# ikt-luh/Unified-Point-Cloud-Compression

Hardware: AMD Instinct MI355X
Metric: points/sec encode+decode, longdress vox10, 1 GPU; bpp & D1-PSNR parity (higher is better)
Workload: dtype f32

## Files before the change

unified_point_cloud_compression_amd/csrc/pcc_conv.hip:

```cpp
#include <vector>

#include "pcc_common.h"

typedef float f32x16 __attribute__((ext_vector_type(16)));

static constexpr int LDS_LD = 36;
static constexpr int MAXK = 128;
static constexpr int MAXK_T = 512;

enum { MODE_CONV = 0, MODE_GDN = 1, MODE_IGDN = 2 };
#ifdef PCC_DBG_BUILD
#define PCC_DBG_ON(a, bit) (((a).dbg & (bit)) != 0)
#else
#define PCC_DBG_ON(a, bit) false
#endif
__device__ inline float act1(float v, int act, float slope);

struct ConvArgs {
  const float* feat;
  const float* wp;
  const float* bias;
  const int* hdr;
  const int* nbr;
  const int* rows;
  float* out;
  long long n_out;
  long long n_in;
  long long wp_elems;
  const int* pair_in = nullptr;
  const int* tile_k = nullptr;
  const long long* n_tiles = nullptr;
  const unsigned char* featb = nullptr;
  int ksplit = 1;
  float* part = nullptr;
  int dbg = 0;
  int nt = 0;
  bool wh_ok = false;
  const unsigned char* feath = nullptr;
  const float* frow_inv = nullptr;
  int arith = PCC_ARITH_H3;
  int* guard = nullptr;
  float guard_lim = 0.f;
  int cin, cout, cout_pad;
  int cb_log2;
  int ppo;
  int act;
  float slope;
};

__host__ __device__ inline int bn_for(int cout) { return cout >= 128 ? 128 : (cout > 32 ? 64 : 32); }

static constexpr unsigned BUF_OOB = 0xFFFF0000u;
static constexpr long long BUF_MAX_BYTES = 0xFFFE0000ll;

template <int WM, int WN, int TM, int TN, int MODE, bool BUF>
__global__ void __launch_bounds__(256) k_conv_mfma(ConvArgs a) {
  constexpr int BM = WM * TM * 32;
  constexpr int BN = WN * TN * 32;
  static_assert(WM * WN == 4, "4 waves per workgroup");
  __shared__ __attribute__((aligned(16))) float As[BM * LDS_LD];
  __shared__ __attribute__((aligned(16))) float Bs[BN * LDS_LD];
  __shared__ unsigned char act_flag[MAXK];
  __shared__ unsigned char act_list[MAXK];
  __shared__ unsigned char act_kid[MAXK];
  __shared__ int s_nact;

  const int tid = threadIdx.x, lane = tid & 63, w = tid >> 6;

  const int cpx = gridDim.x >> 3;
  const int wid = (blockIdx.x & 7) * cpx + (blockIdx.x >> 3);
  const int gy = a.cout_pad / BN;
  int tile_id = wid / gy;
  int colblock = (wid - tile_id * gy) * BN;
  if (a.hdr == nullptr && a.pair_in == nullptr && gy > 8) {
    const int g = wid / (8 * gy), rem = wid - g * 8 * gy;
    colblock = (rem >> 3) * BN;
    tile_id = g * 8 + (rem & 7);
  }

  int pos0, npos, k_count, koff_begin;
  long long seg_pos_count;
  const int* seg_nbr = nullptr;
  const bool pair_mode = (a.pair_in != nullptr);
  bool identity = (a.hdr == nullptr) && !pair_mode;
  if (pair_mode) {
// ... 3278 lines not shown
    prof_note(PCC_FORM_GATHER_CSR, 0.0, 0.0);
    prof_push();
  }
  return PCC_OK;
}

extern "C" int pcc_convt_fwd_csr(const float* feat_in, int64_t n_in, int32_t cin, const float* packed_w,
                                 const float* bias, int32_t K, int32_t cout, const int32_t* first,
                                 const int32_t* pair_ids, int64_t n_out, float* T, float* out, int32_t act, float slope,
                                 const int32_t* ex_nbr, int32_t ex_K, const float* ex_bias, int32_t arith, int32_t* d_guard,
                                 void* stream) {
  return convt_fwd_csr_impl(feat_in, n_in, cin, packed_w, bias, K, cout, first, pair_ids, n_out, T, out, act, slope, ex_nbr,
                            ex_K, ex_bias, nullptr, nullptr, arith, d_guard, stream);
}

static int ilog2_i(int v) { int l = 0; while ((1 << l) < v) ++l; return l; }
static PccGrid grid_from_host(const uint64_t* bits, const int32_t* rank, const int32_t* h) {
  PccGrid g;
  g.bits = (const unsigned long long*)bits; g.rank = rank;
  for (int i = 0; i < 3; ++i) { g.lo[i] = h[i]; g.dims[i] = h[3 + i]; }
  g.ts_log2 = ilog2_i(h[6]); g.nbatch = h[7];
  return g;
}

extern "C" int pcc_convt_fwd_csr_grid(const float* feat_in, int64_t n_in, int32_t cin, const float* packed_w,
                                      const float* bias, int32_t K, int32_t cout, const int32_t* first,
                                      const int32_t* pair_ids, int64_t n_out, float* T, float* out, int32_t act, float slope,
                                      const int64_t* out_keys, const uint64_t* out_bits, const int32_t* out_rank,
                                      const int32_t* h_out, const float* ex_bias, const int32_t* wg_end, int32_t arith,
                                      int32_t* d_guard, void* stream) {
  PCC_REQUIRE(out_keys && out_bits && out_rank && h_out && ex_bias, "pcc_convt_fwd_csr_grid: NULL array");
  const PccGrid ex = grid_from_host(out_bits, out_rank, h_out);
  return convt_fwd_csr_impl(feat_in, n_in, cin, packed_w, bias, K, cout, first, pair_ids, n_out, T, out, act, slope,
                            nullptr, 27, ex_bias, &ex, (const long long*)out_keys, arith, d_guard, stream, wg_end);
}

struct ThinGridArgs {
  const float* t; const float* bias; const long long* keys; PccGrid g; float* out; long long n; int cout;
};

template <int COUT_MAX>
__global__ void __launch_bounds__(256) k_thin_gather_grid(ThinGridArgs a) {
  const long long p = (long long)blockIdx.x * 256 + threadIdx.x;
  if (p >= a.n) return;
  const PccGrid& g = a.g;
  const long long key = a.keys[p];
  const int b = (int)(key >> 48);
  const int cx = (((int)((key >> 32) & 0xFFFF) - (int)PCC_BIAS - g.lo[0]) >> g.ts_log2);
  const int cy = (((int)((key >> 16) & 0xFFFF) - (int)PCC_BIAS - g.lo[1]) >> g.ts_log2);
  const int cz = (((int)(key & 0xFFFF) - (int)PCC_BIAS - g.lo[2]) >> g.ts_log2);
  const int z_lo = cz > 0 ? cz - 1 : 0, z_hi = cz + 1 < g.dims[2] ? cz + 1 : g.dims[2] - 1;
  const int nz = z_hi - z_lo + 1;
  float acc[COUT_MAX];
#pragma unroll
  for (int o = 0; o < COUT_MAX; ++o) acc[o] = 0.f;
#pragma unroll
  for (int c = 0; c < 9; ++c) {
    const int nx = cx + c % 3 - 1, ny = cy + c / 3 - 1;
    if (nx < 0 || ny < 0 || nx >= g.dims[0] || ny >= g.dims[1]) continue;
    const long long cell = (((long long)b * g.dims[0] + nx) * g.dims[1] + ny) * g.dims[2] + z_lo;
    const long long wi = cell >> 6;
    const int sh = (int)(cell & 63);
    const unsigned long long w0 = g.bits[wi];
    unsigned long long f64 = w0 >> sh;
    if (sh + nz > 64) f64 |= g.bits[wi + 1] << (64 - sh);
    unsigned f = (unsigned)f64 & ((1u << nz) - 1u);
    if (!f) continue;
    int r = g.rank[wi] + __popcll(w0 & ((1ull << sh) - 1ull));
    while (f) {
      const int t = __ffs((int)f) - 1;
      f &= f - 1;
      const int k = c + 9 * (z_lo + t - cz + 1);
#pragma unroll
      for (int o = 0; o < COUT_MAX; ++o)
        if (o < a.cout) acc[o] += a.t[(long long)(k * a.cout + o) * a.n + r];
      ++r;
    }
  }
#pragma unroll
  for (int o = 0; o < COUT_MAX; ++o)
    if (o < a.cout) a.out[p * a.cout + o] = acc[o] + (a.bias ? a.bias[o] : 0.f);
}

__global__ void __launch_bounds__(256) k_thin_gather_grid1(ThinGridArgs a) {
  const long long p = (long long)blockIdx.x * 256 + threadIdx.x;
  if (p >= a.n) return;
  const PccGrid& g = a.g;
  const long long key = a.keys[p];
  const int b = (int)(key >> 48);
  const int cx = (((int)((key >> 32) & 0xFFFF) - (int)PCC_BIAS - g.lo[0]) >> g.ts_log2);
  const int cy = (((int)((key >> 16) & 0xFFFF) - (int)PCC_BIAS - g.lo[1]) >> g.ts_log2);
  const int cz = (((int)(key & 0xFFFF) - (int)PCC_BIAS - g.lo[2]) >> g.ts_log2);
  const int z_lo = cz > 0 ? cz - 1 : 0, z_hi = cz + 1 < g.dims[2] ? cz + 1 : g.dims[2] - 1;
  const int nz = z_hi - z_lo + 1;
  const int dz0 = z_lo - cz + 1;
  unsigned long long w0[9], w1[9];
  int rk[9], sh[9];
  bool ok[9];
#pragma unroll
  for (int c = 0; c < 9; ++c) {
    const int nx = cx + c % 3 - 1, ny = cy + c / 3 - 1;
    ok[c] = !(nx < 0 || ny < 0 || nx >= g.dims[0] || ny >= g.dims[1]);
    const long long cell = ok[c] ? (((long long)b * g.dims[0] + nx) * g.dims[1] + ny) * g.dims[2] + z_lo : 0ll;
    const long long wi = cell >> 6;
    sh[c] = (int)(cell & 63);
    w0[c] = g.bits[wi];
    rk[c] = g.rank[wi];
    w1[c] = (sh[c] + nz > 64) ? g.bits[wi + 1] : 0ull;
  }
  const __amdgpu_buffer_rsrc_t rsT = __builtin_amdgcn_make_buffer_rsrc(const_cast<float*>(a.t), (short)0,
                                                                       (int)(unsigned)((size_t)27 * a.n * 4), 0x00020000);
  float v[27];
#pragma unroll
  for (int c = 0; c < 9; ++c) {
    unsigned long long f64 = w0[c] >> sh[c];
    if (sh[c] + nz > 64) f64 |= w1[c] << (64 - sh[c]);
    const unsigned f = ok[c] ? ((unsigned)f64 & ((1u << nz) - 1u)) : 0u;
    const int r = rk[c] + __popcll(w0[c] & ((1ull << sh[c]) - 1ull));
#pragma unroll
    for (int t = 0; t < 3; ++t) {
      const int k = c + 9 * (dz0 + t);
      const unsigned row = (unsigned)(r + __popc(f & ((1u << t) - 1u)));
      const unsigned off = ((f >> t) & 1u) ? ((unsigned)k * (unsigned)a.n + row) * 4u : BUF_OOB;
      v[c * 3 + t] = __builtin_bit_cast(float, __builtin_amdgcn_raw_buffer_load_b32(rsT, off, 0, 0));
    }
  }
  float acc = 0.f;
#pragma unroll
  for (int i = 0; i < 27; ++i) acc += v[i];
  a.out[p] = acc + (a.bias ? a.bias[0] : 0.f);
}

template <int CIN>
__global__ void __launch_bounds__(256) k_thin_project_z(const float* __restrict__ feat, const long long* __restrict__ keys,
                                                        long long n_in, long long ts, const float* __restrict__ wt,
                                                        float* __restrict__ t) {
  extern __shared__ __attribute__((aligned(16))) float w_s[];
  __shared__ float sd[27][258];
  for (int i = threadIdx.x; i < 27 * CIN; i += 256) w_s[i] = wt[i];
  __syncthreads();
  const long long base = (long long)blockIdx.x * 256;
  const long long i = base + threadIdx.x;
  const bool valid = i < n_in;
  float4 x[CIN / 4];
#pragma unroll
  for (int c = 0; c < CIN / 4; ++c) x[c] = valid ? reinterpret_cast<const float4*>(feat + i * CIN)[c] : make_float4(0.f, 0.f, 0.f, 0.f);
  const long long key = valid ? keys[i] : -(1ll << 62);
  const bool adjm = valid && i > 0 && keys[i - 1] == key - ts;
  const bool adjp = valid && i + 1 < n_in && keys[i + 1] == key + ts;
#pragma unroll 1
  for (int k = 0; k < 27; ++k) {
    float acc = 0.f;
#pragma unroll
    for (int c = 0; c < CIN / 4; ++c) {
      const float4 w = reinterpret_cast<const float4*>(w_s + k * CIN)[c];
      acc += x[c].x * w.x + x[c].y * w.y + x[c].z * w.z + x[c].w * w.w;
    }
    sd[k][1 + threadIdx.x] = acc;
  }
  if (threadIdx.x < 18) {
    const int e = threadIdx.x < 9 ? threadIdx.x : threadIdx.x - 9;
    const long long r = threadIdx.x < 9 ? base - 1 : base + 256;
    const int k = threadIdx.x < 9 ? e : e + 18;
    float acc = 0.f;
    if (r >= 0 && r < n_in) {
#pragma unroll
      for (int c = 0; c < CIN / 4; ++c) {
        const float4 xv = reinterpret_cast<const float4*>(feat + r * CIN)[c];
        const float4 w = reinterpret_cast<const float4*>(w_s + k * CIN)[c];
        acc += xv.x * w.x + xv.y * w.y + xv.z * w.z + xv.w * w.w;
      }
    }
    sd[k][threadIdx.x < 9 ? 0 : 257] = acc;
  }
  __syncthreads();
  if (!valid) return;
  const int col = 1 + threadIdx.x;
#pragma unroll 1
  for (int g = 0; g < 9; ++g) {
    const float lo = sd[g][col], mid = sd[g + 9][col], hi = sd[g + 18][col];
    const float from_dn = sd[g][col - 1];
    const float from_up = sd[g + 18][col + 1];
    t[(long long)g * n_in + i] = (mid + (adjm ? from_dn : 0.f)) + (adjp ? from_up : 0.f);
    t[(long long)(9 + g) * n_in + i] = lo;
    t[(long long)(18 + g) * n_in + i] = hi;
  }
}

__global__ void __launch_bounds__(256) k_thin_gather_grid1z(ThinGridArgs a) {
  const long long p = (long long)blockIdx.x * 256 + threadIdx.x;
  if (p >= a.n) return;
  const PccGrid& g = a.g;
  const long long key = a.keys[p];
  const int b = (int)(key >> 48);
  const int cx = (((int)((key >> 32) & 0xFFFF) - (int)PCC_BIAS - g.lo[0]) >> g.ts_log2);
  const int cy = (((int)((key >> 16) & 0xFFFF) - (int)PCC_BIAS - g.lo[1]) >> g.ts_log2);
  const int cz = (((int)(key & 0xFFFF) - (int)PCC_BIAS - g.lo[2]) >> g.ts_log2);
  const int z_lo = cz > 0 ? cz - 1 : 0, z_hi = cz + 1 < g.dims[2] ? cz + 1 : g.dims[2] - 1;
  const int nz = z_hi - z_lo + 1;
  const int dz0 = z_lo - cz + 1;
  unsigned long long w0[9], w1[9];
  int rk[9], sh[9];
  bool ok[9];
#pragma unroll
  for (int c = 0; c < 9; ++c) {
    const int nx = cx + c % 3 - 1, ny = cy + c / 3 - 1;
    ok[c] = !(nx < 0 || ny < 0 || nx >= g.dims[0] || ny >= g.dims[1]);
    const long long cell = ok[c] ? (((long long)b * g.dims[0] + nx) * g.dims[1] + ny) * g.dims[2] + z_lo : 0ll;
    const long long wi = cell >> 6;
    sh[c] = (int)(cell & 63);
    w0[c] = g.bits[wi];
    rk[c] = g.rank[wi];
    w1[c] = (sh[c] + nz > 64) ? g.bits[wi + 1] : 0ull;
  }
  const __amdgpu_buffer_rsrc_t rsT = __builtin_amdgcn_make_buffer_rsrc(const_cast<float*>(a.t), (short)0,
                                                                       (int)(unsigned)((size_t)27 * a.n * 4), 0x00020000);
  const int tm = 1 - dz0;
  float v[27];
#pragma unroll
  for (int c = 0; c < 9; ++c) {
    unsigned long long f64 = w0[c] >> sh[c];
    if (sh[c] + nz > 64) f64 |= w1[c] << (64 - sh[c]);
    const unsigned f = ok[c] ? ((unsigned)f64 & ((1u << nz) - 1u)) : 0u;
    const unsigned r = (unsigned)(rk[c] + __popcll(w0[c] & ((1ull << sh[c]) - 1ull)));
    const bool mid = (f >> tm) & 1u;
    const bool low = dz0 == 0 && (f & 1u);
    const int tu = 2 - dz0;
    const bool upp = tu < nz && ((f >> tu) & 1u);
    const unsigned row_mid = r + __popc(f & ((1u << tm) - 1u));
    const unsigned row_up = r + __popc(f & ((1u << tu) - 1u));
    const unsigned n = (unsigned)a.n;
    const unsigned o_s = mid ? ((unsigned)c * n + row_mid) * 4u : BUF_OOB;
    const unsigned o_u = (!mid && low) ? ((unsigned)(9 + c) * n + r) * 4u : BUF_OOB;
    const unsigned o_d = (!mid && upp) ? ((unsigned)(18 + c) * n + row_up) * 4u : BUF_OOB;
    v[c * 3 + 0] = __builtin_bit_cast(float, __builtin_amdgcn_raw_buffer_load_b32(rsT, o_s, 0, 0));
    v[c * 3 + 1] = __builtin_bit_cast(float, __builtin_amdgcn_raw_buffer_load_b32(rsT, o_u, 0, 0));
    v[c * 3 + 2] = __builtin_bit_cast(float, __builtin_amdgcn_raw_buffer_load_b32(rsT, o_d, 0, 0));
  }
  float acc = 0.f;
#pragma unroll
  for (int i = 0; i < 27; ++i) acc += v[i];
  a.out[p] = acc + (a.bias ? a.bias[0] : 0.f);
}

static long long g_thin_z_min_rows = 1ll << 20;
extern "C" int pcc_set_thin_z_min_rows(int64_t rows) { g_thin_z_min_rows = rows; return PCC_OK; }

extern "C" size_t pcc_thin_grid_ws_bytes(int64_t n, int32_t cout) { return (size_t)27 * cout * (size_t)(n > 0 ? n : 1) * sizeof(float) + 256; }

extern "C" int pcc_conv_thin_grid_fwd(const float* feat, int64_t n, int32_t cin, const float* packed_w ,
                                      const float* bias, int32_t cout, const int64_t* keys, const uint64_t* bits,
                                      const int32_t* rank, const int32_t* h_grid, float* out, void* ws, size_t ws_bytes,
                                      void* stream) {
  hipStream_t s = (hipStream_t)stream;
  if (n <= 0) return PCC_OK;
  PCC_REQUIRE(feat && packed_w && keys && bits && rank && h_grid && out && ws, "pcc_conv_thin_grid_fwd: NULL array");
  PCC_REQUIRE(cout >= 1 && cout <= 4 && conv_kind(27, cin, cout) == KIND_THIN_T, "pcc_conv_thin_grid_fwd: unsupported shape cin=%d cout=%d", cin, cout);
  if (ws_bytes < pcc_thin_grid_ws_bytes(n, cout)) { pcc_set_error("pcc_conv_thin_grid_fwd: workspace too small"); return PCC_EWS; }
  float* t = (float*)ws;
  const int kc = 27 * cout;
  if (g_thin_z_min_rows >= 0 && cout == 1 && cin == 16 && (size_t)27 * n * 4 <= (size_t)BUF_MAX_BYTES && n >= g_thin_z_min_rows) {
    k_thin_project_z<16><<<(unsigned)pcc_cdiv(n, 256), 256, (size_t)27 * 16 * sizeof(float), s>>>(
        feat, (const long long*)keys, n, (long long)h_grid[6], packed_w, t);
    ThinGridArgs az;
    az.t = t; az.bias = bias; az.keys = (const long long*)keys; az.g = grid_from_host(bits, rank, h_grid); az.out = out; az.n = n; az.cout = 1;
    k_thin_gather_grid1z<<<(unsigned)pcc_cdiv(n, 256), 256, 0, s>>>(az);
    PCC_LAUNCH_CHECK();
    return PCC_OK;
  }
  switch (cin) {
    case 4: PCC_TRY(launch_project<4>(feat, n, packed_w, kc, t, s)); break;
    case 8: PCC_TRY(launch_project<8>(feat, n, packed_w, kc, t, s)); break;
    case 16: PCC_TRY(launch_project<16>(feat, n, packed_w, kc, t, s)); break;
    case 32: PCC_TRY(launch_project<32>(feat, n, packed_w, kc, t, s)); break;
    default: PCC_TRY(launch_project<64>(feat, n, packed_w, kc, t, s)); break;
  }
  ThinGridArgs a;
  a.t = t; a.bias = bias; a.keys = (const long long*)keys; a.g = grid_from_host(bits, rank, h_grid); a.out = out; a.n = n; a.cout = cout;
  if (cout == 1 && (size_t)27 * n * 4 <= (size_t)BUF_MAX_BYTES) k_thin_gather_grid1<<<(unsigned)pcc_cdiv(n, 256), 256, 0, s>>>(a);
  else if (cout == 1) k_thin_gather_grid<1><<<(unsigned)pcc_cdiv(n, 256), 256, 0, s>>>(a);
  else k_thin_gather_grid<4><<<(unsigned)pcc_cdiv(n, 256), 256, 0, s>>>(a);
  PCC_LAUNCH_CHECK();
  return PCC_OK;
}

__global__ void k_gdn_pack(const float* __restrict__ beta_raw, const float* __restrict__ gamma_raw, int c,
                           float beta_bound, float gamma_bound, float pedestal, int cout_pad, int cb_log2,
                           float* __restrict__ packed, float* __restrict__ beta_eff) {
  const long long t = (long long)blockIdx.x * blockDim.x + threadIdx.x;
  if (t < c) {
    const float b = fmaxf(beta_raw[t], beta_bound);
    beta_eff[t] = b * b - pedestal;
  }
  const long long total = (long long)c * cout_pad;
  if (t >= total) return;
  const int CB = 1 << cb_log2;
  const int within = (int)(t & (CB - 1));
  const long long q = t >> cb_log2;
  const int col = (int)(q % cout_pad);
  const int cbi = (int)(q / cout_pad);
  const int ci = (cbi << cb_log2) + within;
  float v = 0.f;
  if (col < c) {
    const float g = fmaxf(gamma_raw[(long long)col * c + ci], gamma_bound);
    v = g * g - pedestal;
  }
  packed[t] = v;
// ... 54 lines not shown
```

unified_point_cloud_compression_amd/csrc/pcc_map.hip:

```cpp
#include <string.h>

#include "pcc_common.h"

struct SegPlan {
  int nseg;
  int K;
  int listed;
  int k_count[PCC_MAP_MAX_SEG];
  int koff_begin[PCC_MAP_MAX_SEG];
  unsigned char koffs[192];
  unsigned char order[192];
};

__device__ __forceinline__ void write_hdr(const SegPlan& plan, const int* __restrict__ class_begin, int class_stride,
                                          int64_t n_out, int* __restrict__ hdr) {
  {
    const int i = (int)threadIdx.x;
    if (i < plan.K && i < 192) {
      hdr[HDR_KOFFS + i] = plan.listed ? plan.koffs[i] : i;
      hdr[HDR_ORDER + i] = plan.order[i];
    }
  }
  if (threadIdx.x != 0) return;
  hdr[HDR_NSEG] = plan.nseg;
  hdr[HDR_K] = plan.K;
  hdr[HDR_FLAGS] = plan.listed;
  int64_t nbr_begin = 0;
  for (int s = 0; s < plan.nseg; ++s) {
    int pb = 0, pc = (int)n_out;
    if (class_begin) {
      pb = class_begin[s * class_stride];
      const int pe = (s + 1 < plan.nseg) ? class_begin[(s + 1) * class_stride] : (int)n_out;
      pc = pe - pb;
    }
    int* seg = hdr + HDR_SEG0 + s * SEG_WORDS;
    seg[SEG_POS_BEGIN] = pb;
    seg[SEG_POS_COUNT] = pc;
    seg[SEG_K_COUNT] = plan.k_count[s];
    seg[SEG_KOFF_BEGIN] = plan.koff_begin[s];
    seg[SEG_NBR_LO] = (int)(nbr_begin & 0xFFFFFFFFll);
    seg[SEG_NBR_HI] = (int)(nbr_begin >> 32);
    nbr_begin += (int64_t)pc * plan.k_count[s];
  }
}

__global__ void k_write_hdr(SegPlan plan, const int* __restrict__ class_begin, int class_stride,
                            int64_t n_out, int* __restrict__ hdr) {
  if (blockIdx.x != 0) return;
  write_hdr(plan, class_begin, class_stride, n_out, hdr);
}

static constexpr bool ORDER_Z_INNERMOST = false;
static void plan_order(SegPlan& plan, int ks) {
  for (int s = 0; s < plan.nseg; ++s) {
    const int kb = plan.koff_begin[s], kc = plan.k_count[s];
    int key[192];
    for (int j = 0; j < kc; ++j) {
      const int kid = plan.listed ? plan.koffs[kb + j] : (kb + j);
      key[j] = (kid % (ks * ks)) * ks + kid / (ks * ks);
      plan.order[kb + j] = (unsigned char)j;
    }
    if (!ORDER_Z_INNERMOST) continue;
    for (int a = 1; a < kc; ++a)
      for (int b = a; b > 0 && key[plan.order[kb + b]] < key[plan.order[kb + b - 1]]; --b) {
        const unsigned char t = plan.order[kb + b]; plan.order[kb + b] = plan.order[kb + b - 1]; plan.order[kb + b - 1] = t;
      }
  }
}

__device__ inline void count_pairs(bool hit, int* __restrict__ block_counts) {
  if (!block_counts) return;
  __shared__ int wc[4];
  const unsigned long long m = __ballot(hit);
  if ((threadIdx.x & 63) == 0) wc[threadIdx.x >> 6] = __popcll(m);
  __syncthreads();
  if (threadIdx.x == 0)
    block_counts[(int64_t)blockIdx.y * gridDim.x + blockIdx.x] = wc[0] + wc[1] + wc[2] + wc[3];
}

__global__ void __launch_bounds__(1024) k_sum_counts(const int* __restrict__ c, int64_t n,
                                                     int64_t* __restrict__ total) {
  __shared__ long long ws[16];
  long long s = 0;
  for (int64_t i = threadIdx.x; i < n; i += 1024) s += c[i];
#pragma unroll
// ... 529 lines not shown
  return PCC_OK;
}

extern "C" int pcc_coords_stride_grid(const int64_t* keys, int64_t n, const int64_t* d_n, const int32_t* h_grid, uint64_t* bits,
                                      int32_t* rank, int64_t* out_keys, int64_t* d_count, void* ws, size_t ws_bytes,
                                      void* stream) {
  hipStream_t s = (hipStream_t)stream;
  PCC_REQUIRE(h_grid && bits && rank && out_keys && d_count, "pcc_coords_stride_grid: NULL array");
  const int64_t words = pcc_grid_words(h_grid);
  PCC_REQUIRE(words >= 1 && words < (1ll << 31), "pcc_coords_stride_grid: lattice too large (%lld words)", (long long)words);
  const int P = h_grid[6];
  PCC_REQUIRE(P >= 1 && (P & (P - 1)) == 0, "pcc_coords_stride_grid: pitch must be a power of two");
  PCC_REQUIRE(h_grid[0] % P == 0 && h_grid[1] % P == 0 && h_grid[2] % P == 0,
              "pcc_coords_stride_grid: lattice origin must be a multiple of the pitch %d", P);
  if (ws_bytes < pcc_grid_ws_bytes(words)) {
    pcc_set_error("pcc_coords_stride_grid: workspace too small");
    return PCC_EWS;
  }
  PCC_CHECK_HIP(hipMemsetAsync(bits, 0, (size_t)words * 8, s));
  if (n > 0) {
    PCC_REQUIRE(keys, "pcc_coords_stride_grid: keys is NULL");
    k_grid_bits_any<<<(unsigned)pcc_cdiv(n, 256), 256, 0, s>>>(keys, n, d_n, h_grid[0], h_grid[1], h_grid[2], h_grid[3],
                                                              h_grid[4], h_grid[5], ilog2(P), (unsigned long long*)bits);
    PCC_LAUNCH_CHECK();
  }
  return grid_rank((const unsigned long long*)bits, words, rank, h_grid, ilog2(P), out_keys, d_count, ws, ws_bytes, s);
}

__global__ void k_grid_bits_each(const int64_t* __restrict__ keys, int64_t n, int lo0, int lo1, int lo2, int d0, int d1,
                                 int d2, int tsl, unsigned long long* __restrict__ bits, int64_t* __restrict__ off_lattice) {
  const int64_t i = (int64_t)blockIdx.x * blockDim.x + threadIdx.x;
  if (i >= n) return;
  const int64_t key = keys[i];
  const int x = (int)((key >> 32) & 0xFFFF) - (int)PCC_BIAS - lo0, y = (int)((key >> 16) & 0xFFFF) - (int)PCC_BIAS - lo1,
            z = (int)(key & 0xFFFF) - (int)PCC_BIAS - lo2;
  if ((x | y | z) & ((1 << tsl) - 1)) { *off_lattice = 1; return; }
  const long long c = grid_cell(key, lo0, lo1, lo2, d0, d1, d2, tsl);
  atomicOr(&bits[c >> 6], 1ull << (c & 63));
}

__global__ void k_grid_first_user(const int64_t* __restrict__ keys, int64_t n, int lo0, int lo1, int lo2, int d0, int d1,
                                  int d2, int tsl, const unsigned long long* __restrict__ bits,
                                  const int* __restrict__ rank, int* __restrict__ first_user) {
  const int64_t i = (int64_t)blockIdx.x * blockDim.x + threadIdx.x;
  if (i >= n) return;
  const long long c = grid_cell(keys[i], lo0, lo1, lo2, d0, d1, d2, tsl);
  const unsigned long long w = bits[c >> 6];
  const int r = rank[c >> 6] + __popcll(w & ((1ull << (c & 63)) - 1ull));
  atomicMin(&first_user[r], (int)i);
}

extern "C" int pcc_keys_canonicalize_grid(const int64_t* keys, int64_t n, const int32_t* h_grid, uint64_t* bits,
                                          int32_t* rank, int64_t* out_keys, int32_t* first_user, int64_t* d_count,
                                          void* ws, size_t ws_bytes, void* stream) {
  hipStream_t s = (hipStream_t)stream;
  PCC_REQUIRE(keys && h_grid && bits && rank && out_keys && first_user && d_count && n > 0 && n < (1ll << 31),
              "pcc_keys_canonicalize_grid: bad arguments");
  const int64_t words = pcc_grid_words(h_grid);
  PCC_REQUIRE(words >= 1 && words < (1ll << 31), "pcc_keys_canonicalize_grid: lattice too large (%lld words)", (long long)words);
  const int P = h_grid[6];
  PCC_REQUIRE(P >= 1 && (P & (P - 1)) == 0, "pcc_keys_canonicalize_grid: pitch must be a power of two");
  if (ws_bytes < pcc_grid_ws_bytes(words)) { pcc_set_error("pcc_keys_canonicalize_grid: workspace too small"); return PCC_EWS; }
  const int tsl = ilog2(P);
  unsigned long long* b = (unsigned long long*)bits;
  PCC_CHECK_HIP(hipMemsetAsync(bits, 0, (size_t)words * 8, s));
  PCC_CHECK_HIP(hipMemsetAsync(first_user, 0x7F, (size_t)n * 4, s));
  PCC_CHECK_HIP(hipMemsetAsync(d_count, 0, 2 * sizeof(int64_t), s));
  const unsigned g = (unsigned)pcc_cdiv(n, 256);
  k_grid_bits_each<<<g, 256, 0, s>>>(keys, n, h_grid[0], h_grid[1], h_grid[2], h_grid[3], h_grid[4], h_grid[5], tsl, b,
                                     d_count + 1);
  PCC_LAUNCH_CHECK();
  PCC_TRY(grid_rank(b, words, rank, h_grid, tsl, out_keys, d_count, ws, ws_bytes, s));
  k_grid_first_user<<<g, 256, 0, s>>>(keys, n, h_grid[0], h_grid[1], h_grid[2], h_grid[3], h_grid[4], h_grid[5], tsl, b,
                                      rank, first_user);
  PCC_LAUNCH_CHECK();
  return PCC_OK;
}

template <int KS>
__global__ void __launch_bounds__(256) k_expand_mark(const int64_t* __restrict__ keys, int64_t n, int ts_out, int lo0,
                                                     int lo1, int lo2, int d0, int d1, int d2, int tsl,
                                                     unsigned long long* __restrict__ bits) {
  const int64_t i = (int64_t)blockIdx.x * blockDim.x + threadIdx.x;
  if (i >= n) return;
  constexpr int H = (KS & 1) ? (KS - 1) / 2 : 0;
  const int kxy = blockIdx.y;
  const int64_t key = keys[i];
  const int b = (int)(key >> 48);
  const int cx = ((int)((key >> 32) & 0xFFFF) - (int)PCC_BIAS - lo0 + (kxy % KS - H) * ts_out) >> tsl;
  const int cy = ((int)((key >> 16) & 0xFFFF) - (int)PCC_BIAS - lo1 + (kxy / KS - H) * ts_out) >> tsl;
  const int cz = ((int)(key & 0xFFFF) - (int)PCC_BIAS - lo2 - H * ts_out) >> tsl;
  const long long cell = (((long long)b * d0 + cx) * d1 + cy) * d2 + cz;
  const int bit = (int)(cell & 63);
  const unsigned long long m = (1ull << KS) - 1ull;
  atomicOr(&bits[cell >> 6], m << bit);
  if (bit + KS > 64) atomicOr(&bits[(cell >> 6) + 1], m >> (64 - bit));
}

struct ExpandCsrArgs {
  const int64_t* out_keys; long long n_out;
  PccGrid in;
  int ts_out; int K;
  int* first;
  int* pair_ids;
  int zk;
  long long* d_total;
};

template <int KS>
struct CsrCols {
  int c0x, c0y, c0z, i0x, i0y, i0z, nx, ny, nz;
  int step, b;
  __device__ __forceinline__ int cell(int ax, int j) const { return (ax == 0 ? c0x : ax == 1 ? c0y : c0z) + j; }
  __device__ __forceinline__ int idx(int ax, int j) const { return (ax == 0 ? i0x : ax == 1 ? i0y : i0z) - step * j; }
  __device__ __forceinline__ int cnt(int ax) const { return ax == 0 ? nx : ax == 1 ? ny : nz; }
  __device__ __forceinline__ void set(int ax, int c0, int i0, int n) {
    if (ax == 0) { c0x = c0; i0x = i0; nx = n; } else if (ax == 1) { c0y = c0; i0y = i0; ny = n; } else { c0z = c0; i0z = i0; nz = n; }
  }
};

template <int KS>
__device__ __forceinline__ void csr_columns(const ExpandCsrArgs& a, long long o, CsrCols<KS>& c) {
  constexpr int H = (KS & 1) ? (KS - 1) / 2 : 0;
  const int64_t key = a.out_keys[o];
  c.b = (int)(key >> 48);
  const int p[3] = {(int)((key >> 32) & 0xFFFF) - (int)PCC_BIAS - a.in.lo[0],
                    (int)((key >> 16) & 0xFFFF) - (int)PCC_BIAS - a.in.lo[1],
                    (int)(key & 0xFFFF) - (int)PCC_BIAS - a.in.lo[2]};
  const int tm = (1 << a.in.ts_log2) - 1;
  c.step = (1 << a.in.ts_log2) / a.ts_out;
  if ((KS & 1) && a.ts_out * 2 == (1 << a.in.ts_log2)) {
    const int tl = a.in.ts_log2 - 1;
#pragma unroll
    for (int ax = 0; ax < 3; ++ax) {
      const int P = p[ax] >> tl;
      int c0 = (P - H + 1) >> 1, c1 = (P + H) >> 1;
      c0 = c0 < 0 ? 0 : c0;
      c1 = c1 >= a.in.dims[ax] ? a.in.dims[ax] - 1 : c1;
      const int m = c1 - c0 + 1;
      c.set(ax, c0, P + H - 2 * c0, (m > 0 && !(p[ax] & (a.ts_out - 1))) ? m : 0);
    }
    return;
  }
#pragma unroll
  for (int ax = 0; ax < 3; ++ax) {
    int m = 0, c0 = 0, i0 = 0;
#pragma unroll
    for (int ia = KS - 1; ia >= 0; --ia) {
      const int rel = p[ax] - (ia - H) * a.ts_out;
      const int cc = rel >> a.in.ts_log2;
      if (rel >= 0 && !(rel & tm) && cc < a.in.dims[ax]) {
        if (m == 0) { c0 = cc; i0 = ia; }
        ++m;
      }
    }
    c.set(ax, c0, i0, m);
  }
}

__device__ __forceinline__ unsigned csr_field(const unsigned long long* __restrict__ bits, long long cell, int nz, long long* word,
                                              unsigned long long* w0_out) {
  const long long wi = cell >> 6;
  const int sh = (int)(cell & 63);
  const unsigned long long w0 = bits[wi];
  unsigned long long f = w0 >> sh;
  if (sh + nz > 64) f |= bits[wi + 1] << (64 - sh);
  *word = wi;
  *w0_out = w0;
  return (unsigned)f & ((1u << nz) - 1u);
}

template <int KS, int M>
__global__ void __launch_bounds__(256) k_expand_csr_count(ExpandCsrArgs a) {
  const long long o = (long long)blockIdx.x * blockDim.x + threadIdx.x;
  if (o >= a.n_out) return;
  CsrCols<KS> c;
  csr_columns<KS>(a, o, c);
  int total = 0;
  if (c.b < a.in.nbatch && c.cnt(2) > 0) {
// ... 14 lines not shown
        for (int jy = 0; jy < M; ++jy) {
          const int jx = jx0 + gx;
          const bool ok = jx < c.cnt(0) && jy < c.cnt(1);
          const long long cell = ok ? cell00 + jx * slab + (long long)jy * a.in.dims[2] : 0ll;
          const long long dw = cell >> 5, dw2 = dw < last_dw ? dw : last_dw;
          sh[gx * M + jy] = ok ? (int)(cell & 31) + 32 * (int)(dw - dw2) : 64;
          const unsigned lo = bits32[dw2], hi = bits32[dw2 + 1];
          w[gx * M + jy] = (unsigned long long)lo | ((unsigned long long)hi << 32);
        }
#pragma unroll
      for (int i = 0; i < G * M; ++i) total += sh[i] < 64 ? __popc((unsigned)(w[i] >> (sh[i] & 63)) & fmask) : 0;
    }
  }
  a.first[o] = total;
  if (o == a.n_out - 1) a.first[a.n_out] = 0;
}

template <int KS, typename F>
__device__ __forceinline__ void csr_probe(const ExpandCsrArgs& a, long long o, F&& on_hit) {
  CsrCols<KS> c;
  csr_columns<KS>(a, o, c);
  if (c.b >= a.in.nbatch || c.cnt(2) == 0) return;
  constexpr int MY = KS == 7 ? 4 : KS;
  const unsigned* const bits32 = reinterpret_cast<const unsigned*>(a.in.bits);
  const long long cells = (long long)a.in.nbatch * a.in.dims[0] * a.in.dims[1] * a.in.dims[2];
  const long long last_w = ((cells + 63) >> 6) - 1;
  const unsigned fmask = (1u << c.cnt(2)) - 1u;
  const int kzs = a.zk ? 1 : KS * KS;
  const long long cell00 = (((long long)c.b * a.in.dims[0] + c.cell(0, 0)) * a.in.dims[1] + c.cell(1, 0)) * a.in.dims[2] + c.cell(2, 0);
  const long long slab = (long long)a.in.dims[1] * a.in.dims[2];
  for (int jx = 0; jx < c.cnt(0); ++jx) {
    unsigned long long w0[MY];
    unsigned nx[MY];
    int rk[MY], sh[MY];
#pragma unroll
    for (int jy = 0; jy < MY; ++jy) {
      const bool ok = jy < c.cnt(1);
      const long long cell = ok ? cell00 + jx * slab + (long long)jy * a.in.dims[2] : 0ll;
      const long long wi = cell >> 6;
      sh[jy] = ok ? (int)(cell & 63) : 64;
      w0[jy] = a.in.bits[wi];
      nx[jy] = bits32[2 * (wi < last_w ? wi + 1 : last_w)];
      rk[jy] = a.in.rank[wi];
    }
#pragma unroll
    for (int jy = 0; jy < MY; ++jy) {
      if (sh[jy] >= 64) continue;
      unsigned long long win = w0[jy] >> sh[jy];
      if (sh[jy]) win |= (unsigned long long)nx[jy] << (64 - sh[jy]);
      unsigned f = (unsigned)win & fmask;
      if (!f) continue;
      int i = rk[jy] + __popcll(w0[jy] & ((1ull << sh[jy]) - 1ull));
      const int kxy = a.zk ? KS * (c.idx(1, jy) + KS * c.idx(0, jx)) : c.idx(0, jx) + KS * c.idx(1, jy);
      while (f) {
        const int t = __ffs((int)f) - 1;
        f &= f - 1;
        on_hit(i, kxy + kzs * c.idx(2, t));
        ++i;
      }
    }
  }
}

template <int KS>
__global__ void __launch_bounds__(256) k_expand_csr_fill(ExpandCsrArgs a) {
  constexpr int CAP = 256 * 20;
  __shared__ int stage[CAP];
  const long long o0 = (long long)blockIdx.x * blockDim.x;
  const long long o = o0 + threadIdx.x;
  const long long o_end = min(a.n_out, o0 + 256);
  const int base = a.first[o0], total = a.first[o_end] - base;
  const bool staged = total <= CAP;
  if (a.d_total && blockIdx.x == 0 && threadIdx.x == 0) *a.d_total = a.first[a.n_out];
  if (o < a.n_out) {
    int wpos = a.first[o] - base;
    if (staged) csr_probe<KS>(a, o, [&](int i, int kidx) { stage[wpos++] = i * a.K + kidx; });
    else { wpos += base; csr_probe<KS>(a, o, [&](int i, int kidx) { a.pair_ids[wpos++] = i * a.K + kidx; }); }
  }
  if (!staged) return;
  __syncthreads();
  for (int t = threadIdx.x; t < total; t += 256) a.pair_ids[base + t] = stage[t];
}

template <int KS>
__global__ void __launch_bounds__(256) k_expand_csr_slot(ExpandCsrArgs a, int slot, int* __restrict__ wg_end) {
  constexpr int R = 12;
  __shared__ int region[256 * R];
  __shared__ int wsum[4];
  const long long o = (long long)blockIdx.x * 256 + threadIdx.x;
  int cnt = 0;
  int* const mine = region + threadIdx.x;
  if (o < a.n_out) csr_probe<KS>(a, o, [&](int i, int kidx) { if (cnt < R) mine[cnt * 256] = i * a.K + kidx; ++cnt; });
  const int lane = threadIdx.x & 63, w = threadIdx.x >> 6;
  int inc = cnt;
#pragma unroll
  for (int d = 1; d < 64; d <<= 1) { const int t = __shfl_up(inc, d); if (lane >= d) inc += t; }
  if (lane == 63) wsum[w] = inc;
  __syncthreads();
  int off = inc - cnt, total = 0;
#pragma unroll
  for (int q = 0; q < 4; ++q) { const int sv = wsum[q]; if (q < w) off += sv; total += sv; }
  const int base = (int)blockIdx.x * slot;
  if (threadIdx.x == 0) {
    wg_end[blockIdx.x] = base + total;
    if (a.d_total) atomicAdd((unsigned long long*)a.d_total, (unsigned long long)total);
  }
  if (o >= a.n_out) return;
  a.first[o] = base + off;
  int* const dst = a.pair_ids + base + off;
  if (cnt <= R) { for (int j = 0; j < cnt; ++j) dst[j] = mine[j * 256]; }
  else { int wpos = 0; csr_probe<KS>(a, o, [&](int i, int kidx) { dst[wpos++] = i * a.K + kidx; }); }
}

__global__ void k_set_int(int* p, int v) { *p = v; }

extern "C" int pcc_coords_expand_grid(const int64_t* keys, int64_t n, int32_t kernel_size, const int32_t* h_out,
                                      uint64_t* bits, int32_t* rank, int64_t* out_keys, int64_t* d_count, void* ws,
                                      size_t ws_bytes, void* stream) {
  hipStream_t s = (hipStream_t)stream;
  PCC_REQUIRE(keys && h_out && bits && rank && out_keys && d_count && n > 0, "pcc_coords_expand_grid: bad arguments");
  PCC_REQUIRE(kernel_size == 2 || kernel_size == 3 || kernel_size == 5, "pcc_coords_expand_grid: kernel_size %d unsupported", kernel_size);
  const int64_t words = pcc_grid_words(h_out);
  PCC_REQUIRE(words >= 1 && words < (1ll << 31), "pcc_coords_expand_grid: lattice too large (%lld words)", (long long)words);
  const int ts_out = h_out[6];
  PCC_REQUIRE(ts_out >= 1 && (ts_out & (ts_out - 1)) == 0, "pcc_coords_expand_grid: pitch must be a power of two");
  if (ws_bytes < pcc_grid_ws_bytes(words)) { pcc_set_error("pcc_coords_expand_grid: workspace too small"); return PCC_EWS; }
  PCC_CHECK_HIP(hipMemsetAsync(bits, 0, (size_t)words * 8, s));
  const dim3 g((unsigned)pcc_cdiv(n, 256), (unsigned)(kernel_size * kernel_size));
  unsigned long long* b = (unsigned long long*)bits;
  const int tsl = ilog2(ts_out);
  if (kernel_size == 2) k_expand_mark<2><<<g, 256, 0, s>>>(keys, n, ts_out, h_out[0], h_out[1], h_out[2], h_out[3], h_out[4], h_out[5], tsl, b);
  else if (kernel_size == 3) k_expand_mark<3><<<g, 256, 0, s>>>(keys, n, ts_out, h_out[0], h_out[1], h_out[2], h_out[3], h_out[4], h_out[5], tsl, b);
  else k_expand_mark<5><<<g, 256, 0, s>>>(keys, n, ts_out, h_out[0], h_out[1], h_out[2], h_out[3], h_out[4], h_out[5], tsl, b);
  PCC_LAUNCH_CHECK();
  return grid_rank(b, words, rank, h_out, tsl, out_keys, d_count, ws, ws_bytes, s);
}

extern "C" size_t pcc_expand_grid_csr_ws_bytes(int64_t n_out) { return pcc_scan_ws_bytes(n_out + 1) + 256; }

static int expand_grid_csr(const int64_t* out_keys, int64_t n_out, int32_t kernel_size, int32_t ts_out,
                           const uint64_t* in_bits, const int32_t* in_rank, const int32_t* h_in,
                           int64_t n_in, int32_t* first, int32_t* pair_ids, int64_t* d_total, void* ws, size_t ws_bytes, int zk,
                           void* stream);
extern "C" int pcc_coords_expand_grid_csr(const int64_t* out_keys, int64_t n_out, int32_t kernel_size, int32_t ts_out,
                                          const uint64_t* in_bits, const int32_t* in_rank, const int32_t* h_in,
                                          int64_t n_in, int32_t* first, int32_t* pair_ids, int64_t* d_total, void* ws,
                                          size_t ws_bytes, void* stream) {
  return expand_grid_csr(out_keys, n_out, kernel_size, ts_out, in_bits, in_rank, h_in, n_in, first, pair_ids, d_total, ws, ws_bytes, 0, stream);
}
extern "C" int pcc_coords_expand_grid_csr_zk(const int64_t* out_keys, int64_t n_out, int32_t kernel_size, int32_t ts_out,
                                             const uint64_t* in_bits, const int32_t* in_rank, const int32_t* h_in,
                                             int64_t n_in, int32_t* first, int32_t* pair_ids, int64_t* d_total, void* ws,
                                             size_t ws_bytes, void* stream) {
  return expand_grid_csr(out_keys, n_out, kernel_size, ts_out, in_bits, in_rank, h_in, n_in, first, pair_ids, d_total, ws, ws_bytes, 1, stream);
}
static int expand_grid_csr(const int64_t* out_keys, int64_t n_out, int32_t kernel_size, int32_t ts_out,
                           const uint64_t* in_bits, const int32_t* in_rank, const int32_t* h_in,
                           int64_t n_in, int32_t* first, int32_t* pair_ids, int64_t* d_total, void* ws, size_t ws_bytes, int zk,
                           void* stream) {
  hipStream_t s = (hipStream_t)stream;
  PCC_REQUIRE(out_keys && in_bits && in_rank && h_in && first && pair_ids && n_out > 0, "pcc_coords_expand_grid_csr: bad arguments");
  PCC_REQUIRE(kernel_size == 2 || kernel_size == 3 || kernel_size == 5 || kernel_size == 7,
              "pcc_coords_expand_grid_csr: kernel_size %d unsupported", kernel_size);
  const int K = kernel_size * kernel_size * kernel_size;
  PCC_REQUIRE(n_in * K < (1ll << 31), "pcc_coords_expand_grid_csr: too many pairs");
  if (ws_bytes < pcc_expand_grid_csr_ws_bytes(n_out)) { pcc_set_error("pcc_coords_expand_grid_csr: workspace too small"); return PCC_EWS; }
  ExpandCsrArgs a;
  a.out_keys = out_keys; a.n_out = n_out; a.ts_out = ts_out; a.K = K; a.first = first; a.pair_ids = pair_ids; a.zk = zk;
  a.d_total = (long long*)d_total;
  a.in.bits = (const unsigned long long*)in_bits; a.in.rank = in_rank;
  for (int i = 0; i < 3; ++i) { a.in.lo[i] = h_in[i]; a.in.dims[i] = h_in[3 + i]; }
  a.in.ts_log2 = ilog2(h_in[6]); a.in.nbatch = h_in[7];
  const unsigned g = (unsigned)pcc_cdiv(n_out, 256);
  PCC_REQUIRE(ts_out >= 1 && h_in[6] >= ts_out && h_in[6] % ts_out == 0, "pcc_coords_expand_grid_csr: input pitch %d is not a multiple of the output pitch %d", h_in[6], ts_out);
  const bool same_pitch = h_in[6] == ts_out;
// ... 112 lines not shown
```

Baseline: 54.88 million.

## Share occupancy-bitmap fetches across wave lanes in the same z-column run

```diff
diff --git a/unified_point_cloud_compression_amd/csrc/pcc_conv.hip b/unified_point_cloud_compression_amd/csrc/pcc_conv.hip
--- a/unified_point_cloud_compression_amd/csrc/pcc_conv.hip
+++ b/unified_point_cloud_compression_amd/csrc/pcc_conv.hip
@@ -1,6 +1,7 @@
 #include <vector>
 
 #include "pcc_common.h"
+#include "pcc_zrun.h"
 
 typedef float f32x16 __attribute__((ext_vector_type(16)));
 
@@ -3445,41 +3446,93 @@
     if (o < a.cout) a.out[p * a.cout + o] = acc[o] + (a.bias ? a.bias[o] : 0.f);
 }
 
-__global__ void __launch_bounds__(256) k_thin_gather_grid1(ThinGridArgs a) {
-  const long long p = (long long)blockIdx.x * 256 + threadIdx.x;
-  if (p >= a.n) return;
-  const PccGrid& g = a.g;
-  const long long key = a.keys[p];
+__device__ __forceinline__ void thin_fields(const PccGrid& g, const long long* __restrict__ keys, long long p, bool valid,
+                                            ZrunRec* wave_recs, unsigned (&f)[9], unsigned (&r)[9], int* nz_out, int* dz0_out) {
+  const long long key = valid ? keys[p] : -1ll;
   const int b = (int)(key >> 48);
   const int cx = (((int)((key >> 32) & 0xFFFF) - (int)PCC_BIAS - g.lo[0]) >> g.ts_log2);
   const int cy = (((int)((key >> 16) & 0xFFFF) - (int)PCC_BIAS - g.lo[1]) >> g.ts_log2);
   const int cz = (((int)(key & 0xFFFF) - (int)PCC_BIAS - g.lo[2]) >> g.ts_log2);
   const int z_lo = cz > 0 ? cz - 1 : 0, z_hi = cz + 1 < g.dims[2] ? cz + 1 : g.dims[2] - 1;
   const int nz = z_hi - z_lo + 1;
-  const int dz0 = z_lo - cz + 1;
-  unsigned long long w0[9], w1[9];
-  int rk[9], sh[9];
-  bool ok[9];
-#pragma unroll
-  for (int c = 0; c < 9; ++c) {
-    const int nx = cx + c % 3 - 1, ny = cy + c / 3 - 1;
-    ok[c] = !(nx < 0 || ny < 0 || nx >= g.dims[0] || ny >= g.dims[1]);
-    const long long cell = ok[c] ? (((long long)b * g.dims[0] + nx) * g.dims[1] + ny) * g.dims[2] + z_lo : 0ll;
-    const long long wi = cell >> 6;
-    sh[c] = (int)(cell & 63);
-    w0[c] = g.bits[wi];
-    rk[c] = g.rank[wi];
-    w1[c] = (sh[c] + nz > 64) ? g.bits[wi + 1] : 0ull;
-  }
+  *nz_out = nz;
+  *dz0_out = z_lo - cz + 1;
+  const int chunk0 = (z_lo >> ZRUN_CHUNK_LOG2) << ZRUN_CHUNK_LOG2;
+  const ZrunSeg sg = zrun_segments(valid ? ((key & ~0xFFFFll) | (long long)(z_lo >> ZRUN_CHUNK_LOG2)) : -1ll);
+#pragma unroll
+  for (int c = 0; c < 9; ++c) { f[c] = 0u; r[c] = 0u; }
+  if (sg.nseg > 4 * ZRUN_SEGS) {
+    if (!valid) return;
+    unsigned long long w0[9], w1[9];
+    int rk[9], sh[9];
+    bool ok[9];
+#pragma unroll
+    for (int c = 0; c < 9; ++c) {
+      const int nx = cx + c % 3 - 1, ny = cy + c / 3 - 1;
+      ok[c] = !(nx < 0 || ny < 0 || nx >= g.dims[0] || ny >= g.dims[1]);
+      const long long cell = ok[c] ? (((long long)b * g.dims[0] + nx) * g.dims[1] + ny) * g.dims[2] + z_lo : 0ll;
+      const long long wi = cell >> 6;
+      sh[c] = (int)(cell & 63);
+      w0[c] = g.bits[wi];
+      rk[c] = g.rank[wi];
+      w1[c] = (sh[c] + nz > 64) ? g.bits[wi + 1] : 0ull;
+    }
+#pragma unroll
+    for (int c = 0; c < 9; ++c) {
+      unsigned long long f64 = w0[c] >> sh[c];
+      if (sh[c] + nz > 64) f64 |= w1[c] << (64 - sh[c]);
+      f[c] = ok[c] ? ((unsigned)f64 & ((1u << nz) - 1u)) : 0u;
+      r[c] = (unsigned)(rk[c] + __popcll(w0[c] & ((1ull << sh[c]) - 1ull)));
+    }
+    return;
+  }
+  const long long cells = (long long)g.nbatch * g.dims[0] * g.dims[1] * g.dims[2];
+  const long long last_w = ((cells + 63) >> 6) - 1;
+  const long long colbase = valid ? (((long long)b * g.dims[0] + cx) * g.dims[1] + cy) * g.dims[2] + chunk0 : 0ll;
+  const unsigned cxy = (unsigned)cx | ((unsigned)cy << 16);
+  const unsigned long long rows = __ballot(valid);
+  zrun_trips(sg, wave_recs,
+    [&](int h, int col) {
+      const int src = h < 0 ? 0 : h;
+      const long long cb = __shfl(colbase, src);
+      const unsigned xy = __shfl(cxy, src);
+      const int dx = col % 3 - 1, dy = col / 3 - 1;
+      const int nx = (int)(xy & 0xFFFFu) + dx, ny = (int)(xy >> 16) + dy;
+      ZrunRec rec = zrun_no_rec();
+      if (h >= 0 && ((rows >> src) & 1ull) && col < 9 && nx >= 0 && ny >= 0 && nx < g.dims[0] && ny < g.dims[1])
+        rec = zrun_fetch(g.bits, g.rank, cb + ((long long)dx * g.dims[1] + dy) * g.dims[2], last_w);
+      return rec;
+    },
+    [&](const ZrunRec* recs) {
+      if (!valid) return;
+      const long long cell0 = colbase + (z_lo - chunk0);
+#pragma unroll
+      for (int c = 0; c < 9; ++c) {
+        const int nx = cx + c % 3 - 1, ny = cy + c / 3 - 1;
+        const bool ok = !(nx < 0 || ny < 0 || nx >= g.dims[0] || ny >= g.dims[1]);
+        const long long cell = cell0 + ((long long)(c % 3 - 1) * g.dims[1] + (c / 3 - 1)) * g.dims[2];
+        int row;
+        const unsigned long long win = zrun_window(recs[c], ok ? cell : cell0, z_lo - chunk0, &row);
+        f[c] = ok ? ((unsigned)win & ((1u << nz) - 1u)) : 0u;
+        r[c] = (unsigned)row;
+      }
+    });
+}
+
+__global__ void __launch_bounds__(256) k_thin_gather_grid1(ThinGridArgs a) {
+  __shared__ ZrunRec recs[4][PCC_WAVE];
+  const long long p = (long long)blockIdx.x * 256 + threadIdx.x;
+  unsigned f9[9], r9[9];
+  int nz, dz0;
+  thin_fields(a.g, a.keys, p, p < a.n, recs[threadIdx.x >> 6], f9, r9, &nz, &dz0);
+  if (p >= a.n) return;
   const __amdgpu_buffer_rsrc_t rsT = __builtin_amdgcn_make_buffer_rsrc(const_cast<float*>(a.t), (short)0,
                                                                        (int)(unsigned)((size_t)27 * a.n * 4), 0x00020000);
   float v[27];
 #pragma unroll
   for (int c = 0; c < 9; ++c) {
-    unsigned long long f64 = w0[c] >> sh[c];
-    if (sh[c] + nz > 64) f64 |= w1[c] << (64 - sh[c]);
-    const unsigned f = ok[c] ? ((unsigned)f64 & ((1u << nz) - 1u)) : 0u;
-    const int r = rk[c] + __popcll(w0[c] & ((1ull << sh[c]) - 1ull));
+    const unsigned f = f9[c];
+    const int r = (int)r9[c];
 #pragma unroll
     for (int t = 0; t < 3; ++t) {
       const int k = c + 9 * (dz0 + t);
@@ -3551,41 +3604,19 @@
 }
 
 __global__ void __launch_bounds__(256) k_thin_gather_grid1z(ThinGridArgs a) {
+  __shared__ ZrunRec recs[4][PCC_WAVE];
   const long long p = (long long)blockIdx.x * 256 + threadIdx.x;
+  unsigned f9[9], r9[9];
+  int nz, dz0;
+  thin_fields(a.g, a.keys, p, p < a.n, recs[threadIdx.x >> 6], f9, r9, &nz, &dz0);
   if (p >= a.n) return;
-  const PccGrid& g = a.g;
-  const long long key = a.keys[p];
-  const int b = (int)(key >> 48);
-  const int cx = (((int)((key >> 32) & 0xFFFF) - (int)PCC_BIAS - g.lo[0]) >> g.ts_log2);
-  const int cy = (((int)((key >> 16) & 0xFFFF) - (int)PCC_BIAS - g.lo[1]) >> g.ts_log2);
-  const int cz = (((int)(key & 0xFFFF) - (int)PCC_BIAS - g.lo[2]) >> g.ts_log2);
-  const int z_lo = cz > 0 ? cz - 1 : 0, z_hi = cz + 1 < g.dims[2] ? cz + 1 : g.dims[2] - 1;
-  const int nz = z_hi - z_lo + 1;
-  const int dz0 = z_lo - cz + 1;
-  unsigned long long w0[9], w1[9];
-  int rk[9], sh[9];
-  bool ok[9];
-#pragma unroll
-  for (int c = 0; c < 9; ++c) {
-    const int nx = cx + c % 3 - 1, ny = cy + c / 3 - 1;
-    ok[c] = !(nx < 0 || ny < 0 || nx >= g.dims[0] || ny >= g.dims[1]);
-    const long long cell = ok[c] ? (((long long)b * g.dims[0] + nx) * g.dims[1] + ny) * g.dims[2] + z_lo : 0ll;
-    const long long wi = cell >> 6;
-    sh[c] = (int)(cell & 63);
-    w0[c] = g.bits[wi];
-    rk[c] = g.rank[wi];
-    w1[c] = (sh[c] + nz > 64) ? g.bits[wi + 1] : 0ull;
-  }
   const __amdgpu_buffer_rsrc_t rsT = __builtin_amdgcn_make_buffer_rsrc(const_cast<float*>(a.t), (short)0,
                                                                        (int)(unsigned)((size_t)27 * a.n * 4), 0x00020000);
   const int tm = 1 - dz0;
   float v[27];
 #pragma unroll
   for (int c = 0; c < 9; ++c) {
-    unsigned long long f64 = w0[c] >> sh[c];
-    if (sh[c] + nz > 64) f64 |= w1[c] << (64 - sh[c]);
-    const unsigned f = ok[c] ? ((unsigned)f64 & ((1u << nz) - 1u)) : 0u;
-    const unsigned r = (unsigned)(rk[c] + __popcll(w0[c] & ((1ull << sh[c]) - 1ull)));
+    const unsigned f = f9[c], r = r9[c];
     const bool mid = (f >> tm) & 1u;
     const bool low = dz0 == 0 && (f & 1u);
     const int tu = 2 - dz0;
diff --git a/unified_point_cloud_compression_amd/csrc/pcc_map.hip b/unified_point_cloud_compression_amd/csrc/pcc_map.hip
--- a/unified_point_cloud_compression_amd/csrc/pcc_map.hip
+++ b/unified_point_cloud_compression_amd/csrc/pcc_map.hip
@@ -1,6 +1,7 @@
 #include <string.h>
 
 #include "pcc_common.h"
+#include "pcc_zrun.h"
 
 struct SegPlan {
   int nseg;
@@ -696,10 +697,10 @@
                                                      int lo1, int lo2, int d0, int d1, int d2, int tsl,
                                                      unsigned long long* __restrict__ bits) {
   const int64_t i = (int64_t)blockIdx.x * blockDim.x + threadIdx.x;
-  if (i >= n) return;
+  const bool valid = i < n;
   constexpr int H = (KS & 1) ? (KS - 1) / 2 : 0;
   const int kxy = blockIdx.y;
-  const int64_t key = keys[i];
+  const int64_t key = valid ? keys[i] : 0;
   const int b = (int)(key >> 48);
   const int cx = ((int)((key >> 32) & 0xFFFF) - (int)PCC_BIAS - lo0 + (kxy % KS - H) * ts_out) >> tsl;
   const int cy = ((int)((key >> 16) & 0xFFFF) - (int)PCC_BIAS - lo1 + (kxy / KS - H) * ts_out) >> tsl;
@@ -707,8 +708,12 @@
   const long long cell = (((long long)b * d0 + cx) * d1 + cy) * d2 + cz;
   const int bit = (int)(cell & 63);
   const unsigned long long m = (1ull << KS) - 1ull;
-  atomicOr(&bits[cell >> 6], m << bit);
-  if (bit + KS > 64) atomicOr(&bits[(cell >> 6) + 1], m >> (64 - bit));
+  const long long wi = valid ? cell >> 6 : -1ll;
+  const ZrunSeg sg = zrun_segments(wi);
+  bool last;
+  const unsigned long long all = zrun_or_reduce(sg, valid ? m << bit : 0ull, &last);
+  if (last && valid) atomicOr(&bits[wi], all);
+  if (valid && bit + KS > 64) atomicOr(&bits[wi + 1], m >> (64 - bit));
 }
 
 struct ExpandCsrArgs {
@@ -889,15 +894,69 @@
   for (int t = threadIdx.x; t < total; t += 256) a.pair_ids[base + t] = stage[t];
 }
 
+template <int KS, typename F>
+__device__ __forceinline__ void csr_probe_zrun(const ExpandCsrArgs& a, long long o, bool valid, ZrunRec* wave_recs, F&& on_hit) {
+  static_assert(KS == 5 || KS == 7, "4 x 4 columns per segment");
+  CsrCols<KS> c;
+  c.c0x = c.c0y = c.c0z = c.i0x = c.i0y = c.i0z = c.nx = c.ny = c.nz = c.step = c.b = 0;
+  if (valid) csr_columns<KS>(a, o, c);
+  const bool live = valid && c.b < a.in.nbatch && c.nx > 0 && c.ny > 0 && c.nz > 0;
+  const int zc = live ? c.c0z : 0;
+  const int chunk0 = (zc >> ZRUN_CHUNK_LOG2) << ZRUN_CHUNK_LOG2;
+  const long long skey = live ? (long long)((a.out_keys[o] & ~0xFFFFll) | (long long)(zc >> ZRUN_CHUNK_LOG2)) : -1ll;
+  const ZrunSeg sg = zrun_segments(skey);
+  if (sg.nseg > 4 * ZRUN_SEGS) {
+    if (live) csr_probe<KS>(a, o, on_hit);
+    return;
+  }
+  const long long cells = (long long)a.in.nbatch * a.in.dims[0] * a.in.dims[1] * a.in.dims[2];
+  const long long last_w = ((cells + 63) >> 6) - 1;
+  const long long slab = (long long)a.in.dims[1] * a.in.dims[2];
+  const long long cell00 = (((long long)c.b * a.in.dims[0] + c.c0x) * a.in.dims[1] + c.c0y) * a.in.dims[2] + zc;
+  const long long base00 = cell00 - (zc - chunk0);
+  const int nxy = live ? (c.nx | (c.ny << 8)) : 0;
+  zrun_trips(sg, wave_recs,
+    [&](int h, int col) {
+      const int src = h < 0 ? 0 : h;
+      const long long cb = __shfl(base00, src);
+      const int nn = __shfl(nxy, src);
+      const int jx = col >> 2, jy = col & 3;
+      ZrunRec r = zrun_no_rec();
+      if (h >= 0 && jx < (nn & 255) && jy < (nn >> 8))
+        r = zrun_fetch(a.in.bits, a.in.rank, cb + jx * slab + (long long)jy * a.in.dims[2], last_w);
+      return r;
+    },
+    [&](const ZrunRec* recs) {
+      const unsigned fmask = (1u << c.nz) - 1u;
+      const int kzs = a.zk ? 1 : KS * KS;
+      for (int jx = 0; jx < c.nx; ++jx)
+        for (int jy = 0; jy < c.ny; ++jy) {
+          const long long cell = cell00 + jx * slab + (long long)jy * a.in.dims[2];
+          int i;
+          const unsigned long long win = zrun_window(recs[jx * 4 + jy], cell, zc - chunk0, &i);
+          unsigned f = (unsigned)win & fmask;
+          if (!f) continue;
+          const int kxy = a.zk ? KS * (c.idx(1, jy) + KS * c.idx(0, jx)) : c.idx(0, jx) + KS * c.idx(1, jy);
+          while (f) {
+            const int t = __ffs((int)f) - 1;
+            f &= f - 1;
+            on_hit(i, kxy + kzs * c.idx(2, t));
+            ++i;
+          }
+        }
+    });
+}
+
 template <int KS>
 __global__ void __launch_bounds__(256) k_expand_csr_slot(ExpandCsrArgs a, int slot, int* __restrict__ wg_end) {
   constexpr int R = 12;
   __shared__ int region[256 * R];
+  __shared__ ZrunRec recs[4][PCC_WAVE];
   __shared__ int wsum[4];
   const long long o = (long long)blockIdx.x * 256 + threadIdx.x;
   int cnt = 0;
   int* const mine = region + threadIdx.x;
-  if (o < a.n_out) csr_probe<KS>(a, o, [&](int i, int kidx) { if (cnt < R) mine[cnt * 256] = i * a.K + kidx; ++cnt; });
+  csr_probe_zrun<KS>(a, o, o < a.n_out, recs[threadIdx.x >> 6], [&](int i, int kidx) { if (cnt < R) mine[cnt * 256] = i * a.K + kidx; ++cnt; });
   const int lane = threadIdx.x & 63, w = threadIdx.x >> 6;
   int inc = cnt;
 #pragma unroll
diff --git a/unified_point_cloud_compression_amd/csrc/pcc_zrun.h b/unified_point_cloud_compression_amd/csrc/pcc_zrun.h
--- /dev/null
+++ b/unified_point_cloud_compression_amd/csrc/pcc_zrun.h
@@ -0,0 +1,91 @@
+#pragma once
+#include "pcc_common.h"
+
+static constexpr int ZRUN_COLS = 16;
+static constexpr int ZRUN_SEGS = PCC_WAVE / ZRUN_COLS;
+static constexpr int ZRUN_CHUNK_LOG2 = 5;
+
+struct ZrunSeg {
+  unsigned long long heads;
+  int seg;
+  int first;
+  int nseg;
+};
+
+__device__ __forceinline__ ZrunSeg zrun_segments(long long key) {
+  const int lane = (int)(threadIdx.x & 63);
+  const long long prev = __shfl_up(key, 1);
+  ZrunSeg s;
+  s.heads = __ballot(lane == 0 || prev != key);
+  const unsigned long long upto = s.heads & (~0ull >> (63 - lane));
+  s.seg = __popcll(upto) - 1;
+  s.first = 63 - __clzll((long long)upto);
+  s.nseg = __popcll(s.heads);
+  return s;
+}
+
+__device__ __forceinline__ void zrun_wave_sync() {
+  __builtin_amdgcn_fence(__ATOMIC_RELEASE, "wavefront");
+  __builtin_amdgcn_wave_barrier();
+  __builtin_amdgcn_fence(__ATOMIC_ACQUIRE, "wavefront");
+}
+
+template <typename Rec, typename Fetch, typename Use>
+__device__ __forceinline__ void zrun_trips(const ZrunSeg& s, Rec* wave_recs, Fetch&& fetch, Use&& use) {
+  const int lane = (int)(threadIdx.x & 63);
+  const int q = lane / ZRUN_COLS, col = lane % ZRUN_COLS;
+  unsigned long long m = s.heads;
+  for (int t = 0; t * ZRUN_SEGS < s.nseg; ++t) {
+    int h = -1;
+#pragma unroll
+    for (int i = 0; i < ZRUN_SEGS; ++i) {
+      const int hi = m ? __ffsll((long long)m) - 1 : -1;
+      m &= m - 1;
+      h = i == q ? hi : h;
+    }
+    wave_recs[lane] = fetch(h, col);
+    zrun_wave_sync();
+    if (s.seg / ZRUN_SEGS == t) use(wave_recs + (s.seg % ZRUN_SEGS) * ZRUN_COLS);
+    zrun_wave_sync();
+  }
+}
+
+__device__ __forceinline__ unsigned long long zrun_or_reduce(const ZrunSeg& s, unsigned long long v, bool* last) {
+  const int lane = (int)(threadIdx.x & 63);
+#pragma unroll
+  for (int d = 1; d < 64; d <<= 1) {
+    const unsigned long long t = __shfl_up(v, d);
+    if (lane - d >= s.first) v |= t;
+  }
+  *last = lane == 63 || (((s.heads >> 1) >> lane) & 1ull);
+  return v;
+}
+
+struct ZrunRec { unsigned long long w0, w1; int rk; int pad; };
+__device__ __forceinline__ ZrunRec zrun_no_rec() {
+  ZrunRec r;
+  r.w0 = 0ull; r.w1 = 0ull; r.rk = 0; r.pad = 0;
+  return r;
+}
+__device__ __forceinline__ ZrunRec zrun_fetch(const unsigned long long* __restrict__ bits, const int* __restrict__ rank,
+                                              long long cell, long long last_w) {
+  const long long wi = cell >> 6;
+  ZrunRec r;
+  r.w0 = bits[wi];
+  r.w1 = bits[wi < last_w ? wi + 1 : last_w];
+  r.rk = rank[wi];
+  r.pad = 0;
+  return r;
+}
+__device__ __forceinline__ unsigned long long zrun_window(const ZrunRec& r, long long cell, int back, int* row) {
+  const int sh = (int)(cell & 63);
+  const unsigned long long below = (1ull << sh) - 1ull;
+  if ((cell >> 6) == ((cell - back) >> 6)) {
+    *row = r.rk + __popcll(r.w0 & below);
+    unsigned long long win = r.w0 >> sh;
+    if (sh) win |= r.w1 << (64 - sh);
+    return win;
+  }
+  *row = r.rk + __popcll(r.w0) + __popcll(r.w1 & below);
+  return r.w1 >> sh;
+}
```

Measured after the change: 54.68 million. No clear change (-0.4%).
